# BurntSushi/rust-snappy

Hardware: AMD Instinct MI355X
Metric: GiB/s uncompressed (compress + decompress) on zflat/uflat corpus (higher is better)
Workload: dtype u8

## Files before the change

rust-snappy_amd/csrc/snapmi_api.hip:

```cpp
#include <hip/hip_runtime.h>

#include <cstdarg>
#include <cstdio>
#include <cstdlib>
#include <cstring>
#include <new>
#include <string>
#include <vector>

#include "snapmi.h"
#include "snapmi_test.h"
#include "snapmi_ctx.hpp"
#include "snapmi_launch.hpp"
#include "snapmi_device.hpp"
#include "snapmi_kernels.hpp"

using namespace snapmi;

namespace {

void set_err(snapmi_error *e, int kind, uint64_t a = 0, uint64_t b = 0,
             uint64_t c = 0)
{
    if (e) {
// ... 251 lines not shown
        ctx->lane_table_tries = (uint32_t)value;
    else if (strcmp(name, "lane_table_budget_pct") == 0 && value >= 1 &&
             value <= 90)
        ctx->lane_table_budget_pct = (uint32_t)value;
    else if (strcmp(name, "token_pool_pct") == 0 && value >= 1 &&
             value <= 100) {
        ctx->token_pool_pct = (uint32_t)value;
        ctx->token_pool_now = 0;
    } else if (strcmp(name, "token_pool_min_pages") == 0 && value >= 0 &&
               value <= 0x7FFFFFFF)
        ctx->token_pool_min_pages = (uint32_t)value;
    else if (strcmp(name, "span_schedule") == 0 && value >= 0 && value <= 2)
        ctx->span_schedule = (int)value;
    else if (strcmp(name, "lane_coresident") == 0 && value >= 0 && value <= 1)
        ctx->lane_coresident = (int)value;
    else if (strcmp(name, "lane_coresident_min_blocks") == 0 && value >= 1)
        ctx->lane_coresident_min_blocks = (uint64_t)value;
    else if (strcmp(name, "small_table_kernel") == 0 && value >= 0 &&
             value <= 1)
        ctx->small_table_kernel = (int)value;
    else if (strcmp(name, "small_table_min_blocks") == 0 && value >= 1)
        ctx->small_table_min_blocks = (uint64_t)value;
    else if (strcmp(name, "small_batch_kernel") == 0 && value >= 0 &&
             value <= 2)
        ctx->small_batch_kernel = (int)value;
    else if (strcmp(name, "lane_speculate") == 0 && value >= 0 && value <= 1)
        ctx->lane_speculate = (int)value;
    else if (strcmp(name, "lane_tail_probes") == 0 && value >= 0 &&
             value <= 4)
        ctx->lane_tail_probes = (uint32_t)value;
    else if (strcmp(name, "lane_tail_idle_pct") == 0 && value >= 0 &&
             value <= 100)
        ctx->lane_tail_idle_pct = (uint32_t)value;
    else if (strcmp(name, "span_kernel") == 0 && value >= kSpanMin &&
             value <= 1)
        ctx->span_kernel = (int)value;
    else if (strcmp(name, "match_kernel") == 0 && value >= 0 && value <= 2)
        ctx->match_kernel = (int)value;
    else if (strcmp(name, "match_spans_ratio_pct") == 0 && value >= 1 &&
             value <= 200)
        ctx->match_spans_ratio_pct = (uint32_t)value;
    else if (strcmp(name, "release_scratch") == 0 && value >= 0 && value <= 1)
        ctx->release_scratch = (int)value;
    else if (strcmp(name, "batch_long_streams") == 0 && value >= 0 &&
             value <= 1)
        ctx->batch_long_streams = (int)value;
    else if (strcmp(name, "both_wave_cus") == 0 && value >= 0 &&
             value <= 4096)
        ctx->both_wave_cus = (uint32_t)value;
    else if (strcmp(name, "tiny_stream_kernel") == 0 && value >= 0 &&
             value <= 1)
        ctx->tiny_stream_kernel = (int)value;
    else if (strcmp(name, "small_stream_kernel") == 0 && value >= 0 &&
             value <= 2)
        ctx->small_stream_kernel = (int)value;
    else if (strcmp(name, "frame_parallel_walk_min") == 0 && value >= 0)
        ctx->frame_parallel_walk_min = (uint64_t)value;
    else if (strcmp(name, "host_copy_kernel") == 0 && value >= 0 && value <= 3)
        ctx->host_copy_kernel = (int)value;
    else if (strcmp(name, "host_encode_slice") == 0 && value >= (1 << 16))
        ctx->host_encode_slice = (uint64_t)value;
    else if (strcmp(name, "host_decode_slice_chunks") == 0 && value >= 1)
        ctx->host_decode_slice_chunks = (uint64_t)value;
    else if (strcmp(name, "host_batch_slice") == 0 && value >= (1 << 16))
        ctx->host_batch_slice = (uint64_t)value;
    else if (strcmp(name, "range_scratch_bytes") == 0 && value >= (128 << 10))
// ... 42 lines not shown
             value <= 1)
        ctx->lane_table_probe = value != 0;
    else if (strcmp(name, "lane_tables_renew") == 0 && value == 1) {
        if (ctx->lane_tables.p) {
            HIP_TRY(ctx, hipStreamSynchronize(ctx->stream));
            snapmi::free_lane_tables(ctx);
        }
    } else if (strcmp(name, "lane_epoch_preset") == 0 && value >= -1 &&
             value <= 0xFFFF)
        ctx->lane_epoch_preset = value;
    else if (strcmp(name, "index_build_route") == 0 && value >= 0 &&
             value <= 2)
        ctx->index_build_route = (uint32_t)value;
    else if (strcmp(name, "index_build_group_streams") == 0 && value >= 1 &&
             value <= 4096)
        ctx->index_build_group_streams = (uint32_t)value;
    else if (strcmp(name, "stream_seg_log2") == 0 &&
             (value == 0 || value == 10 || value == 12))
        ctx->stream_seg_log2 = (uint32_t)value;
    else if (strcmp(name, "stream_scan_segs") == 0 &&
             (value == 0 || value == 8 || value == 16 || value == 32 ||
              value == 64))
        ctx->stream_scan_segs = (uint32_t)value;
    else if (strcmp(name, "lds_order_ok") == 0 && value >= 0 && value <= 1)
        ctx->lds_order_ok = ctx->lds_order_hw && value != 0;
    else if (strcmp(name, "host_batch_direct_min") == 0 && value >= 0)
        ctx->host_batch_direct_min = (uint64_t)value;
    else if (strcmp(name, "host_batch_pack_to_host") == 0 && value >= 0 &&
             value <= 1)
        ctx->host_batch_pack_to_host = (int)value;
    else if (strcmp(name, "host_batch_listed") == 0 && value >= 0 &&
             value <= 1)
        ctx->host_batch_listed = (int)value;
    else
        return fail_ctx(ctx, SNAPMI_E_ARGUMENT, "unknown test option %s",
                        name);
    return SNAPMI_OK;
}
#endif

void *snapmi_host_alloc(size_t bytes)
{
    void *p = nullptr;
    if (hipHostMalloc(&p, bytes ? bytes : 1, hipHostMallocDefault) != hipSuccess) {
        (void)hipGetLastError();
        return nullptr;
    }
    return p;
}

void snapmi_host_free(void *p)
{
    if (p)
        (void)hipHostFree(p);
}

const char *snapmi_table_probe_log(const snapmi_ctx *ctx)
{
    return ctx ? ctx->probe_log.c_str() : "";
}

size_t snapmi_error_string(const snapmi_error *e, char *buf, size_t cap)
{
    char tmp[256];
    const unsigned long long a = e ? e->a : 0, b = e ? e->b : 0,
                             c = e ? e->c : 0;
// ... 153 lines not shown
        return SNAPMI_TOO_BIG;
    }
    *result = (size_t)v;
    return SNAPMI_OK;
}

int snapmi_ctx_get_info(snapmi_ctx *ctx, const char *name, int64_t *value)
{
    if (!ctx || !name || !value)
        return SNAPMI_E_ARGUMENT;
    if (strcmp(name, "scratch_bytes") == 0) {
        uint64_t sum = ctx->lane_tables.cap;
        for (const DevBuf *b : ctx->dev_bufs)
            sum += b->cap;
        *value = (int64_t)sum;
    } else if (strcmp(name, "token_scratch_bytes") == 0) {
        *value = (int64_t)(ctx->tokens.cap + ctx->tok_pages.cap +
                           ctx->tok_stage.cap + ctx->ntok.cap);
    } else if (strcmp(name, "token_pool_pages") == 0) {
        *value = ctx->tok_pool_pages_last;
#ifdef SNAPMI_TESTING
    } else if (strcmp(name, "lane_multi_rounds") == 0) {
        uint32_t w = 0;
        if (ctx->tok_pages.p) {
            HIP_TRY(ctx, hipSetDevice(ctx->device));
            HIP_TRY(ctx, hipStreamSynchronize(ctx->stream));
            HIP_TRY(ctx, hipMemcpy(&w,
                                   (const uint32_t *)ctx->tok_pages.p +
                                       snapmi::kTokCtlMultiRounds,
                                   sizeof w, hipMemcpyDeviceToHost));
        }
        *value = w;
#endif
    } else if (strcmp(name, "token_pool_pct_now") == 0) {
        *value = ctx->token_pool_now;
    } else if (strcmp(name, "token_pages_asked") == 0 ||
               strcmp(name, "token_blocks_spilled") == 0) {
        HIP_TRY(ctx, hipSetDevice(ctx->device));
        HIP_TRY(ctx, hipStreamSynchronize(ctx->stream));
        const volatile uint32_t *t = ctx->h_tokstat;
        *value = !t ? 0 : name[6] == 'p' ? t[0] : t[1];
    } else if (strcmp(name, "index_streams_pieced") == 0 ||
               strcmp(name, "index_streams_fallback") == 0) {
        unsigned long long w[3] = {0, 0, 0};
        if (ctx->ix_stats_live && ctx->ix_gate.p) {
            HIP_TRY(ctx, hipSetDevice(ctx->device));
            HIP_TRY(ctx, hipStreamSynchronize(ctx->stream));
            HIP_TRY(ctx, hipMemcpy(w, ctx->ix_gate.p, sizeof w,
                                   hipMemcpyDeviceToHost));
        }
        *value = (int64_t)(name[14] == 'p' ? w[1] : w[2]);
    } else if (strcmp(name, "range_pieces") == 0) {
        *value = (int64_t)ctx->rg_pieces;
    } else if (strcmp(name, "range_ranges_ok") == 0 ||
               strcmp(name, "range_ranges_failed") == 0) {
        unsigned long long w[2] = {0, 0};
        if (ctx->rg_stats_live && ctx->rg_stat.p) {
            HIP_TRY(ctx, hipSetDevice(ctx->device));
            HIP_TRY(ctx, hipStreamSynchronize(ctx->stream));
            HIP_TRY(ctx, hipMemcpy(w, ctx->rg_stat.p, sizeof w,
                                   hipMemcpyDeviceToHost));
        }
        *value = (int64_t)(name[13] == 'o' ? w[0] : w[1]);
    } else if (strcmp(name, "write_blocks") == 0) {
        *value = (int64_t)ctx->wr_blocks;
    } else if (strcmp(name, "write_blocks_decoded") == 0) {
// ... 273 lines not shown
```

rust-snappy_amd/csrc/snapmi_compress.hip:

```cpp
#include <type_traits>

#include "snapmi_device.hpp"
#include "snapmi_kernels.hpp"
#include "snapmi_scan.hpp"
#include "snapmi_span.hpp"

namespace snapmi {

namespace {

__device__ __forceinline__ uint32_t hash32(uint32_t x, uint32_t shift)
{
    return (x * 0x1E35A7BDu) >> shift;
}

struct DeltaTable {
    uint32_t d[448];
};
constexpr DeltaTable make_delta()
{
    DeltaTable t{};
    uint32_t skip = 32, p = 0;
    for (int i = 0; i < 448; i++) {
        t.d[i] = p < 0x100000u ? p : 0x100000u;
// ... 1808 lines not shown
            m.out = (gptr)a.out_ptrs[st];
            a.out_lens[st] = tiny_compress(m, n);
        }
        __syncthreads();
    }
}
}
__global__ __launch_bounds__(64) void k_compress_small512(CompressArgs a)
{
    compress_small<512, 8>(a);
}
__global__ __launch_bounds__(64) void k_compress_small1k(CompressArgs a)
{
    compress_small<1024, 4>(a);
}
__global__ __launch_bounds__(64) void k_compress_small2k(CompressArgs a)
{
    compress_small<2048, 2>(a);
}

__device__ __forceinline__ uint32_t ld32p(gcptr p)
{
    uint32_t v;
    __builtin_memcpy(&v, p, 4);
    return v;
}
__device__ __forceinline__ uint64_t ld64p(gcptr p)
{
    uint64_t v;
    __builtin_memcpy(&v, p, 8);
    return v;
}
namespace {
constexpr uint32_t kLaneRingWords = 64 * 64;
constexpr uint32_t kLaneTokWords = 64 * 16;
template <bool kSpec, bool kTail>
__device__ __forceinline__ void match_blocks(
    const CompressArgs &a, const uint32_t lane, const uint32_t g,
    __attribute__((address_space(3))) uint32_t *const ring,
    __attribute__((address_space(3))) unsigned long long *const tokbuf)
{
    typedef __attribute__((address_space(3))) uint32_t l_tok;
    l_tok *const tbuf = (l_tok *)(tokbuf + lane * 16);
    typedef __attribute__((address_space(3))) uint32_t l_u32;
    typedef __attribute__((address_space(3))) u32x4 l_u32x4;
    typedef __attribute__((address_space(1))) u32x4 g_u32x4;
    l_u32 *const win = ring + lane * 64;

    typedef __attribute__((address_space(1))) unsigned long long g_u64;
    typedef unsigned long long u64x2 __attribute__((ext_vector_type(2)));
    typedef __attribute__((address_space(1))) u64x2 g_entry;
    const uint32_t slot =
        a.lane_chunks ? (g % a.lane_chunks) * a.lane_per_chunk + g / a.lane_chunks
                      : g;
    g_entry *const tab =
        (g_entry *)a.lane_tables + (uint64_t)slot * a.lane_stride;
    unsigned long long epoch = a.lane_epochs[g];
    unsigned long long first8 = 0;
    uint32_t first4b = 0;
    uint32_t nblocks = a.blk_first[a.n_streams];
    if (nblocks > a.host_blocks)
        nblocks = a.host_blocks;
    if (nblocks > a.blk_hi)
        nblocks = a.blk_hi;

    enum : uint32_t {
// ... 105 lines not shown
                out_of_work = true;
            } else {
                uint32_t lo = 0, hi_st = a.n_streams;
                if (b < a.n_streams && a.blk_first[b] == b && a.blk_first[b + 1] > b) {
                    lo = b;
                    hi_st = b + 1;
                }
                while (hi_st - lo > 1) {
                    const uint32_t mid = (lo + hi_st) >> 1;
                    if (a.blk_first[mid] <= b)
                        lo = mid;
                    else
                        hi_st = mid;
                }
                const uint32_t k = b - a.blk_first[lo];
                const uint64_t total = a.in_lens[lo];
                const uint64_t boff = (uint64_t)k * kMaxBlock;
                src = (gcptr)a.in_ptrs[lo] + boff;
                n = total - boff < kMaxBlock ? (uint32_t)(total - boff)
                                             : kMaxBlock;
                spilled = false;
                ntok = 0;
                nexc = 0;
                csize = 0;
                next_emit = 0;
                have = true;
                if (n <= a.cls_lo || n > a.cls_hi) {
                    have = false;
                } else if (n < kMinNonLiteral) {
                    g_tok *const at = tok_at(0);
                    if (!spilled)
                        *at = tok_pack(n, 0, 0);
                    a.ntok[b] = spilled ? kTokSpilled : 1u;
                    a.blk_size[b] = token_bytes(n, 0, 0);
                    have = false;
                } else {
                    first8 = ld64p(src);
                    first4b = ld32p(src + 8);
                    epoch = (epoch + 1) & 0xFFFFu;
                    if (epoch == 0) {
                        for (uint32_t i = 0; i < kMaxTable; i++)
                            tab[i] = (u64x2){0, 0};
                        epoch = 1;
                    }
                    shift = 32 - 8;
                    uint32_t tsize = 256;
                    while (tsize < kMaxTable && tsize < n) {
                        shift--;
                        tsize *= 2;
                    }
                    s_limit = n - kInputMargin;
                    s = 1;
                    s_next = 2;
                    skip = 33;
                    mode = kProbe;
                    mis = (uint32_t)(uintptr_t)src & 127u;
                    src_al = src - mis;
                    hi = 0;
                }
            }
        }
        if ((kTail || kProfTailBuild) && M_need) {
            const uint64_t M_out = __ballot(need && out_of_work);
            if (M_out) {
                if (kTail && lane == (uint32_t)__builtin_ctzll(M_out))
                    atomicAdd(&a.ticket[kTicketIdle],
                              (uint32_t)__builtin_popcountll(M_out));
// ... 269 lines not shown
            s_next = s + step;
            skip += step;
            mode = kProbe;
            if (s_next > s_limit)
                finished = true;
        }
        if (finished)
            flush = flush || (ntok & 31) != 0;
        if (flush) {
            g_u32x4 *to = (g_u32x4 *)tok_at((ntok - 1) & ~31u);
            const l_u32x4 *from = (const l_u32x4 *)tbuf;
            const u32x4 t0 = from[0], t1 = from[1], t2 = from[2], t3 = from[3],
                        t4 = from[4], t5 = from[5], t6 = from[6], t7 = from[7];
            if (!spilled) {
                to[0] = t0; to[1] = t1; to[2] = t2; to[3] = t3;
                to[4] = t4; to[5] = t5; to[6] = t6; to[7] = t7;
            }
        }
        if (finished) {
            if (next_emit < n) {
                const uint32_t tl = n - next_emit;
                g_tok *const at =
                    ntok % 32 ? (g_tok *)a.tok_pool +
                                    (uint64_t)tpage * kTokPage + ntok % kTokPage
                              : tok_at(ntok);
                if (!spilled)
                    *at = tok_pack(tl, 0, 0);
                ntok++;
                if (!tok_fits(tl, 0))
                    exc_put(tok_pack64(tl, 0, 0));
                csize += token_bytes(tl, 0, 0);
            }
            a.ntok[b] = spilled ? kTokSpilled : ntok;
            a.blk_size[b] = csize;
            have = false;
        }
    }
    a.lane_epochs[g] = epoch;
    PROF_TAIL(
    if (a.prof && lane == 0)
        atomicMax(&a.prof[kProfTail + 1], (unsigned long long)wall_clock64());
    )
#ifdef SNAPMI_TESTING
    if (kTail && lane == 0 && multi_rounds)
        atomicAdd(&a.tok_ctl[kTokCtlMultiRounds], multi_rounds);
#endif
}
}

#define SNAPMI_LANE_KERNEL(name, spec, tail)                                  \
    __global__ __launch_bounds__(64) void name(CompressArgs a)                \
    {                                                                         \
        __shared__ __attribute__((aligned(16))) uint32_t ring[kLaneRingWords]; \
        __shared__ __attribute__((aligned(16)))                               \
        unsigned long long tokbuf[kLaneTokWords];                             \
        match_blocks<spec, tail>(                                             \
            a, threadIdx.x, blockIdx.x * 64 + threadIdx.x,                    \
            (__attribute__((address_space(3))) uint32_t *)ring,               \
            (__attribute__((address_space(3))) unsigned long long *)tokbuf);  \
    }
SNAPMI_LANE_KERNEL(k_match_blocks, false, true)
SNAPMI_LANE_KERNEL(k_match_blocks_plain, false, false)
SNAPMI_LANE_KERNEL(k_match_blocks_spec, true, false)
#undef SNAPMI_LANE_KERNEL

namespace {
template <bool kTail>
__device__ __forceinline__ void match_both(
    const CompressArgs &a,
    __attribute__((address_space(3))) uint32_t *const ring,
    __attribute__((address_space(3))) unsigned long long *const tokbuf,
    const lptr16 tables)
{
    const uint32_t lane = threadIdx.x & 63;
    const uint32_t wave = uni(threadIdx.x >> 6);
    if (wave < kBothLaneWaves) {
        match_blocks<false, kTail>(
            a, lane, (blockIdx.x * kBothLaneWaves + wave) * 64 + lane,
            ring + wave * kLaneRingWords, tokbuf + wave * kLaneTokWords);
        return;
    }
    const lptr16 table = tables + (wave - kBothLaneWaves) * kMaxTable;
    const uint32_t tbase = (uint32_t)(uintptr_t)table;
    uint32_t nblocks = a.blk_first[a.n_streams];
    if (nblocks > a.host_blocks)
        nblocks = a.host_blocks;
    if (nblocks > a.blk_hi)
        nblocks = a.blk_hi;
    for (;;) {
        const uint32_t b =
            uni(next_back_ticket(a.ticket, lane, a.blk_lo, nblocks));
        if (b == 0xFFFFFFFFu)
            break;
        compress_one_block_span<false, true>(a, b, lane, table, tbase);
    }
    PROF_TAIL(
    if (a.prof && lane == 0)
        atomicMax(&a.prof[kProfTail + 1], (unsigned long long)wall_clock64());
    )
}
}
#define SNAPMI_BOTH_KERNEL(name, tail)                                        \
    __global__ __launch_bounds__(kBothWaves * 64) void name(CompressArgs a)   \
    {                                                                         \
        __shared__ __attribute__((aligned(16)))                               \
        uint32_t ring[kBothLaneWaves][kLaneRingWords];                        \
        __shared__ __attribute__((aligned(16)))                               \
        unsigned long long tokbuf[kBothLaneWaves][kLaneTokWords];             \
        __shared__ __attribute__((aligned(16)))                               \
        uint16_t tables[kBothWaves - kBothLaneWaves][kMaxTable];              \
        match_both<tail>(                                                     \
            a, (__attribute__((address_space(3))) uint32_t *)&ring[0][0],     \
            (__attribute__((address_space(3))) unsigned long long *)          \
                &tokbuf[0][0],                                                \
            (lptr16)&tables[0][0]);                                           \
    }
SNAPMI_BOTH_KERNEL(k_match_both, true)
SNAPMI_BOTH_KERNEL(k_match_both_plain, false)
#undef SNAPMI_BOTH_KERNEL

__global__ __launch_bounds__(64) void k_encode_tokens(CompressArgs a)
{
    const uint32_t lane = threadIdx.x;
    const uint32_t b = a.blk_lo + blockIdx.x;
    uint32_t nblocks = a.blk_first[a.n_streams];
    if (nblocks > a.host_blocks)
        nblocks = a.host_blocks;
    if (nblocks > a.blk_hi)
        nblocks = a.blk_hi;
    if (b >= nblocks)
        return;
    if (a.ntok[b] >= kTokSpilled)
        return;
    uint32_t lo = 0, hi = a.n_streams;
    if (b < a.n_streams && a.blk_first[b] == b && a.blk_first[b + 1] > b) {
        lo = b;
        hi = b + 1;
    }
    while (hi - lo > 1) {
        const uint32_t mid = (lo + hi) >> 1;
        if (a.blk_first[mid] <= b)
            lo = mid;
        else
            hi = mid;
    }
    const uint32_t st = lo;
    const uint32_t k = b - a.blk_first[st];
    const uint64_t total = a.in_lens[st];
    const uint64_t boff = (uint64_t)k * kMaxBlock;
    gcptr src = (gcptr)a.in_ptrs[st] + boff;
    const uint32_t n =
        total - boff < kMaxBlock ? (uint32_t)(total - boff) : kMaxBlock;
    gptr dst;
    if (k == 0) {
        dst = (gptr)a.out_ptrs[st];
        if (lane == 0) {
            uint64_t v = total;
            uint32_t i = 0;
            while (v >= 0x80) {
                dst[i++] = (uint8_t)v | 0x80;
                v >>= 7;
            }
            dst[i] = (uint8_t)v;
        }
        dst += varint_len(total);
    } else if (a.direct) {
        const uint32_t first = a.blk_first[st];
        const uint64_t nb = (total + kMaxBlock - 1) / kMaxBlock;
        if (first + nb > a.host_blocks)
            return;
        dst = (gptr)a.out_ptrs[st] + varint_len(total) +
              (a.blk_off[b] - a.blk_off[first]);
    } else {
        const uint32_t slot = a.slot_first[st] + k - 1;
        if (slot >= a.host_slots)
            return;
        dst = (gptr)a.scratch + (uint64_t)slot * kSlotBytes;
    }
    TokenSink out;
    out.init(src, n, dst, lane);
    typedef __attribute__((address_space(1))) uint32_t g_tok;
    typedef __attribute__((address_space(1))) unsigned long long g_u64;
    const uint32_t ptab =
        lane < kPageTabStride
            ? a.tok_pages[(uint64_t)(b - a.tok_base) * kPageTabStride + lane]
            : 0;
    const g_tok *const pool = (const g_tok *)a.tok_pool;
    const uint32_t count = a.ntok[b];
    uint32_t pos_base = 0, exc_base = 0;
    uint32_t tnext =
        lane < count ? pool[(uint64_t)rdlane(ptab, 0) * kTokPage + lane] : 0;
    for (uint32_t t0 = 0; t0 < count; t0 += kWave) {
        const uint32_t m = count - t0 < kWave ? count - t0 : kWave;
        uint32_t L = 0, C = 0, O = 0;
        const uint32_t t = tnext;
        if (t0 + kWave < count) {
            const uint32_t pg = rdlane(ptab, (t0 + kWave) / kTokPage);
            if (t0 + kWave + lane < count)
                tnext = pool[(uint64_t)pg * kTokPage +
                             (t0 + kWave) % kTokPage + lane];
        }
        const uint32_t field = (t >> 10) & 63u;
        if (lane < m) {
            L = t & 1023u;
            C = field == kTokLiteral ? 0u : field + 4u;
            O = t >> 16;
        }
        const bool ex = lane < m && field == kTokException;
        const uint64_t E = __builtin_amdgcn_ballot_w64(ex);
        if (E) {
            const uint32_t ei =
                exc_base + __builtin_amdgcn_mbcnt_hi(
                               (uint32_t)(E >> 32),
                               __builtin_amdgcn_mbcnt_lo((uint32_t)E, 0));
            const uint32_t eslot = ei / kExcPage < kExcPagesPerBlock
                                       ? ei / kExcPage
                                       : kExcPagesPerBlock - 1;
            const uint32_t epg = (uint32_t)__builtin_amdgcn_ds_bpermute(
                (int)((kTokPagesPerBlock + eslot) << 2), (int)ptab);
            if (ex) {
                const unsigned long long f =
                    ((const g_u64 *)(pool + (uint64_t)epg * kTokPage))
                        [ei % kExcPage];
                L = (uint32_t)f & 0x1FFFFu;
                C = (uint32_t)(f >> 17) & 0xFFFFu;
                O = (uint32_t)(f >> 33) & 0xFFFFu;
            }
            exc_base += (uint32_t)__builtin_popcountll(E);
        }
        const uint32_t span = L + C;
        const uint32_t incl = wave_inclusive_scan(span);
        const uint32_t P = pos_base + incl - span;
        pos_base += rdlane(incl, kWave - 1);
        out.a = (L & 0xFFFFu) | (O << 16);
        out.b = C | (P << 16);
        out.t = m;
        out.flush();
    }
    if (lane == 0 && !a.direct)
        a.blk_size[b] = out.d;
}

namespace {
__device__ __forceinline__ uint32_t plan_blocks(const CompressArgs &a,
                                                uint32_t i, bool report)
{
    const uint64_t len = a.in_lens[i];
    const uint64_t need = max_compress_len_u64(len);
    if (report)
        a.out_lens[i] = 0;
    if (need == 0) {
        if (report)
            set_error(a.errs, i, SNAPMI_TOO_BIG, len, kMaxInput, 0);
        return 0;
    }
    if (a.out_caps && a.out_caps[i] < need) {
        if (report)
            set_error(a.errs, i, SNAPMI_BUFFER_TOO_SMALL, a.out_caps[i], need,
                      0);
        return 0;
    }
    if (len == 0) {
        if (report) {
            ((gptr)a.out_ptrs[i])[0] = 0;
            a.out_lens[i] = 1;
            set_error(a.errs, i, SNAPMI_OK, 0, 0, 0);
        }
        return 0;
    }
    if (report)
        set_error(a.errs, i, SNAPMI_OK, 0, 0, 0);
    if (len < a.small_limit)
        return 0;
// ... 271 lines not shown
```

rust-snappy_amd/csrc/snapmi_ctx.hpp:

```cpp
#pragma once

#include <hip/hip_runtime.h>

#include <cstdarg>
#include <cstdio>
#include <string>
#include <vector>

#include "snapmi.h"

namespace snapmi {

struct DevBuf {
    void *p = nullptr;
    size_t cap = 0;
    bool listed = false;
};

struct PinBuf {
    void *p = nullptr;
    size_t cap = 0;
    bool listed = false;
};

// ... 26 lines not shown
    std::vector<hipMemGenericAllocationHandle_t> lane_chunks;
    size_t lane_chunk_bytes = 0, lane_va_bytes = 0;
    uint32_t lane_chunk_count = 0, lane_per_chunk = 0;
    uint32_t n_lanes = 0;
    uint64_t lane_stride = 0;
    bool lane_table_spread = true;
    bool lane_tables_top = false;
    int compress_mode = 1;
    int span_schedule = 1;
    snapmi::DevBuf sched;
    int lane_coresident = 1;
    uint64_t lane_coresident_min_blocks = 98304;
    const char *last_kernel = "";
    int small_table_kernel = 1;
    uint64_t small_table_min_blocks = 256;
    int small_batch_kernel = 1;
    int span_kernel = 1;
    uint32_t both_wave_cus = 0;
    int release_scratch = 0;
    int match_kernel = 2;
    uint32_t match_spans_ratio_pct = 90;
    volatile uint32_t *h_ratio = nullptr;
    uint32_t ratio_seq = 0;
    uint32_t token_pool_pct = 39, token_pool_now = 0;
    uint32_t token_pool_min_pages = 32768;
    volatile uint32_t *h_tokstat = nullptr;
    uint32_t tokstat_seq = 0, tokstat_seen = 0;
    uint32_t tok_pages_asked = 0, tok_blocks_spilled = 0;
    uint32_t tok_pool_pages_last = 0;
    int lane_speculate = 1;
    uint64_t lane_speculate_max_blocks = 24576;
    uint32_t lane_tail_probes = 2;
    uint32_t lane_tail_idle_pct = 40;
    int tiny_stream_kernel = 1;
    int small_stream_kernel = 1;
    uint64_t decode_many_min = 1u << 20;
    int lane_overlap_encode = 0;
    int lane_tables_uncached = 0;
    int decode_kernel = 3;
    hipStream_t stream2 = nullptr;
    hipEvent_t ev_fork = nullptr, ev_join = nullptr;
    hipEvent_t ev_crc[2] = {nullptr, nullptr};
    bool frame_crc_side_stream = true;
    snapmi::DevBuf st_in, st_out, st_desc, st_prof, ticket, order;
    snapmi::DevBuf sd_tables, sd_desc;
    int batch_long_streams = 1;
    snapmi::DevBuf bl_modes, bl_list, bl_descs, bl_order;
    snapmi::PinBuf pin_bl;
    snapmi::PinBuf pin_bl2;
    snapmi::DevBuf ix_modes, ix_desc, ix_gate;
    uint64_t ix_seq = 0;
    bool ix_stats_live = false;
    snapmi::DevBuf rg_desc, rg_meta, rg_part, rg_room, rg_stat;
    uint64_t range_scratch_bytes = 1ull << 30;
    uint64_t rg_pieces = 0;
    bool rg_stats_live = false;
    snapmi::DevBuf ib_meta, ib_stat;
    snapmi::PinBuf pin_ib, pin_ibg[2];
    hipEvent_t ev_ib = nullptr, ev_ibg[2] = {nullptr, nullptr};
    bool ev_ib_live = false, ev_ibg_live[2] = {false, false};
    uint64_t ib_groups = 0;
    bool ib_stats_live = false;
    snapmi::DevBuf wr_meta, wr_state, wr_z, wr_slot, wr_room, wr_desc, wr_stat;
    snapmi::PinBuf pin_wr;
    hipEvent_t ev_wr = nullptr;
    bool ev_wr_live = false;
// ... 87 lines not shown
```

rust-snappy_amd/csrc/snapmi_kernels.hpp:

```cpp
#pragma once

#include <hip/hip_runtime.h>
#include <stdint.h>

#include "snapmi.h"
#include "snapmi_tiny.hpp"
#include "snapmi_profile.hpp"
#include "snapmi_streamplan.hpp"
#include "snapmi_blockindex.hpp"

namespace snapmi {

struct CompressArgs {
    const void *const *in_ptrs;
    const uint64_t *in_lens;
    void *const *out_ptrs;
    const uint64_t *out_caps;
    uint64_t *out_lens;
    snapmi_error *errs;
    uint32_t *blk_first;
    uint32_t *slot_first;
    uint32_t *blk_size;
    uint64_t *blk_off;
    uint8_t *scratch;
    uint32_t n_streams;
    uint32_t host_blocks;
    uint32_t host_slots;
    uint32_t *ticket;
    uint32_t *sched;
    uint32_t *tok_pool;
    uint32_t *tok_pages;
    uint32_t *tok_ctl;
    uint32_t tok_pool_pages;
    uint32_t *tok_stage;
    uint32_t tok_stage_waves, tok_stage_wave0;
    uint32_t *ntok;
    uint32_t blk_lo, blk_hi;
    uint32_t tok_base;
    uint32_t direct;
    unsigned long long *lane_tables;
    unsigned long long lane_stride;
    uint32_t lane_chunks, lane_per_chunk;
    uint32_t *lane_epochs;
    uint32_t n_lanes;
    uint32_t lane_depth, lane_tail_depth, lane_tail_idle;
    unsigned long long *prof;
    uint2 *plan_part;
    unsigned long long *scan_part;
    uint32_t small_limit;
    uint32_t cls_lo, cls_hi;
};

constexpr uint32_t kCompressWaves = 5;
constexpr uint32_t kSmallTableWaves = 10;
#define SNAPMI_BOTH_WAVES 6
#define SNAPMI_BOTH_LANE_WAVES 4
constexpr uint32_t kBothWaves = SNAPMI_BOTH_WAVES,
                   kBothLaneWaves = SNAPMI_BOTH_LANE_WAVES;
constexpr uint32_t kMaxTokens = 16416;
constexpr uint32_t kTokPage = 512, kExcPage = 256;
constexpr uint32_t kTokPagesPerBlock = (kMaxTokens + kTokPage - 1) / kTokPage;
constexpr uint32_t kExcPagesPerBlock = 4;
constexpr uint32_t kPageTabStride = 40;
static_assert(kTokPagesPerBlock + kExcPagesPerBlock <= kPageTabStride, "");
constexpr uint32_t kPagesPerSmallBlock = (8192 / 4 + 64 + kTokPage - 1) / kTokPage + 1;
constexpr uint32_t kTokCtlList = 16;
constexpr uint32_t kProfTail = 16, kProfTailLanes = 32;
constexpr uint32_t kTicketIdle = 2;
constexpr uint32_t kTokCtlMultiRounds = 4;
constexpr uint32_t kTokStageWords = kMaxTokens + 2 * (kMaxTokens / 16) + 28;
constexpr uint32_t kTokSpilled = 0xFFFFFFFEu;
constexpr uint32_t kTokLiteral = 61, kTokException = 62;
#if defined(__HIPCC__)
__device__ __forceinline__ bool tok_fits(uint32_t lit, uint32_t copy)
{
    return lit <= 1023u && copy <= 64u;
}
__device__ __forceinline__ uint32_t tok_pack(uint32_t lit, uint32_t copy,
                                             uint32_t offset)
{
    const uint32_t field = copy ? copy - 4u : kTokLiteral;
    return tok_fits(lit, copy) ? (offset << 16) | (field << 10) | lit
                               : kTokException << 10;
}
__device__ __forceinline__ unsigned long long tok_pack64(uint32_t lit,
                                                         uint32_t copy,
                                                         uint32_t offset)
{
    return (unsigned long long)lit | ((unsigned long long)copy << 17) |
           ((unsigned long long)offset << 33);
}
#endif

struct DecompressArgs {
    const void *const *in_ptrs;
    const uint64_t *in_lens;
    void *const *out_ptrs;
    const uint64_t *out_caps;
    uint64_t *out_lens;
    snapmi_error *errs;
    const uint8_t *modes;
    const unsigned long long *gate;
// ... 316 lines not shown
```

rust-snappy_amd/csrc/snapmi_launch.hip:

```cpp
#include <hip/hip_runtime.h>

#include <cstdio>
#include <cstring>
#include <vector>

#include "snapmi.h"
#include "snapmi_test.h"
#include "snapmi_ctx.hpp"
#include "snapmi_launch.hpp"
#include "snapmi_pool.hpp"
#include "snapmi_route.hpp"
#include "snapmi_device.hpp"
#include "snapmi_kernels.hpp"

using namespace snapmi;

namespace snapmi {
static_assert(kRouteCompressWaves == kCompressWaves &&
                  kRouteSmallTableWaves == kSmallTableWaves &&
                  kRouteBothWaves == kBothWaves &&
                  kRouteBothLaneWaves == kBothLaneWaves &&
                  kRouteTinyCompress == kTinyCompress &&
                  kRouteSmallCompress == kSmallCompress,
              "snapmi_route.hpp and snapmi_kernels.hpp disagree");
// ... 259 lines not shown
    a.in_lens = d_in_lens;
    a.out_ptrs = d_out_ptrs;
    a.out_caps = d_out_caps;
    a.out_lens = d_out_lens;
    a.errs = d_errs;
    a.blk_first = (uint32_t *)ctx->blk_first.p;
    a.slot_first = (uint32_t *)ctx->slot_first.p;
    a.blk_size = (uint32_t *)ctx->blk_size.p;
    a.blk_off = (uint64_t *)ctx->blk_off.p;
    a.plan_part = (uint2 *)ctx->plan_part.p;
    a.scan_part = (unsigned long long *)ctx->plan_part.p;
    a.n_streams = (uint32_t)n;
    a.host_blocks = (uint32_t)blocks;
    a.host_slots = (uint32_t)slots;
    a.ticket = (uint32_t *)ctx->ticket.p;
    a.tok_pool = nullptr;
    a.tok_pages = nullptr;
    a.tok_ctl = nullptr;
    a.tok_pool_pages = 0;
    a.tok_stage = nullptr;
    a.tok_stage_waves = 0;
    a.tok_stage_wave0 = 0;
    a.sched = nullptr;
    a.ntok = nullptr;
    a.lane_tables = nullptr;
    a.lane_epochs = nullptr;
    a.lane_stride = kMaxTable;
    a.lane_chunks = 0;
    a.lane_per_chunk = 0;
    a.n_lanes = 0;
    a.lane_depth = 1;
    a.lane_tail_depth = 0;
    a.lane_tail_idle = 0;
    a.tok_base = 0;
    a.small_limit = (uint32_t)small_stream_limit(o);
    a.cls_lo = 0;
    a.cls_hi = kMaxBlock;
    a.direct = route.direct ? 1 : 0;
    if (!route.direct &&
        (rc = reserve(ctx, ctx->slots, (slots + 1) * (size_t)kSlotBytes)))
        return rc;
    a.scratch = (uint8_t *)ctx->slots.p;
    a.blk_lo = 0;
    a.blk_hi = (uint32_t)blocks;
    if (ctx->h_tokstat) {
        const volatile uint32_t *t = ctx->h_tokstat;
        const uint32_t seq = t[3];
        if (seq != ctx->tokstat_seen) {
            ctx->tokstat_seen = seq;
            const uint32_t asked = t[0], spilled = t[1], of = t[2];
            if (t[3] == seq && of) {
                ctx->tok_pages_asked = asked;
                ctx->tok_blocks_spilled = spilled;
                ctx->token_pool_now =
                    snapmi::pool_grow(ctx->token_pool_now, spilled, of);
            }
        }
    }
    if (ctx->token_pool_now < ctx->token_pool_pct)
        ctx->token_pool_now = ctx->token_pool_pct;
    const uint64_t pool_pages =
        snapmi::pool_pages(block_bytes, blocks, route.seg_blocks, route.lanes,
                           ctx->token_pool_now, ctx->token_pool_min_pages);
    const size_t pool_bytes = (size_t)(pool_pages + 1) * kTokPage * 4;
    const size_t stage_bytes =
        (size_t)ctx->num_cus * route.stage_waves * kTokStageWords * 4;
// ... 105 lines not shown
        if (route.window_beside) {
            HIP_TRY(ctx, hipEventRecord(ctx->ev_fork, s));
            HIP_TRY(ctx, hipStreamWaitEvent(ctx->stream2, ctx->ev_fork, 0));
            ws = ctx->stream2;
        }
        if (route.sched) {
            const size_t head = (size_t)(16 + n) * 4;
            const size_t lists = (size_t)2 * (slots + 1) * 4;
            if ((rc = reserve(ctx, ctx->sched, head + lists)))
                return rc;
            HIP_TRY(ctx, hipMemsetAsync(ctx->sched.p, 0, head, ws));
            HIP_TRY(ctx, hipMemsetAsync((uint8_t *)ctx->sched.p + head, 0xFF,
                                        lists, ws));
            a.sched = (uint32_t *)ctx->sched.p;
        }
        launch_window(route, a, ws);
        a.sched = nullptr;
    }
    if (route.tokens) {
        HIP_TRY(ctx, hipEventRecord(ctx->ev[4], s));
        for (uint64_t lo = 0; lo < blocks; lo += route.seg_blocks) {
            const uint64_t hi = lo + route.seg_blocks < blocks
                                    ? lo + route.seg_blocks
                                    : blocks;
            const Segment g = segment(o, route, lo, hi);
            a.tok_base = (uint32_t)lo;
            a.blk_lo = (uint32_t)lo;
            a.blk_hi = (uint32_t)g.mid;
            HIP_TRY(ctx, hipMemsetAsync(ctx->tok_pages.p, 0,
                                        kTokCtlList * 4, s));
            if (route.window == WindowKernel::none)
                HIP_TRY(ctx, hipMemsetAsync(ctx->ticket.p, 0, 64, s));
            a.cls_lo = route.small_grid ? 8192 : 0;
            launch_match(o, route, g, a, s);
            if (route.small_grid) {
                HIP_TRY(ctx, hipMemsetAsync(ctx->ticket.p, 0, 64, s));
                a.cls_lo = 0;
                a.cls_hi = 8192;
                hipLaunchKernelGGL(k_match_spans_8k, dim3(route.small_grid),
                                   dim3(kSmallTableWaves * 64), 0, s, a);
            }
            a.cls_lo = 0;
            a.cls_hi = kMaxBlock;
            if (g.mid < hi) {
                HIP_TRY(ctx, hipEventRecord(ctx->ev_fork, s));
                HIP_TRY(ctx,
                        hipStreamWaitEvent(ctx->stream2, ctx->ev_fork, 0));
                hipLaunchKernelGGL(k_encode_tokens,
                                   dim3((uint32_t)(g.mid - lo)), dim3(64), 0,
                                   ctx->stream2, a);
                HIP_TRY(ctx, hipEventRecord(ctx->ev_join, ctx->stream2));
                a.blk_lo = (uint32_t)g.mid;
                a.blk_hi = (uint32_t)hi;
                HIP_TRY(ctx, hipMemsetAsync(ctx->ticket.p, 0, 64, s));
                launch_match(o, route, g, a, s);
            }
            if (hi == blocks)
                HIP_TRY(ctx, hipEventRecord(ctx->ev[5], s));
            if (route.window_beside) {
                HIP_TRY(ctx, hipEventRecord(ctx->ev_join, ctx->stream2));
                HIP_TRY(ctx, hipStreamWaitEvent(s, ctx->ev_join, 0));
            }
            if (route.direct)
                launch_scan_sizes(a, s);
            hipLaunchKernelGGL(k_encode_tokens,
                               dim3((uint32_t)(hi - a.blk_lo)), dim3(64), 0, s,
                               a);
// ... 173 lines not shown
```

Baseline: 123.8.

## Encode tokens inside the combined match kernel's tail once predecessor sizes are known

After: 124.6, median of 4. Within noise of the previous version (+0.7%).

```diff
diff --git a/rust-snappy_amd/csrc/snapmi_api.hip b/rust-snappy_amd/csrc/snapmi_api.hip
--- a/rust-snappy_amd/csrc/snapmi_api.hip
+++ b/rust-snappy_amd/csrc/snapmi_api.hip
@@ -307,6 +307,8 @@
     else if (strcmp(name, "lane_tail_idle_pct") == 0 && value >= 0 &&
              value <= 100)
         ctx->lane_tail_idle_pct = (uint32_t)value;
+    else if (strcmp(name, "tail_encode") == 0 && value >= 0 && value <= 1)
+        ctx->tail_encode = (int)value;
     else if (strcmp(name, "span_kernel") == 0 && value >= kSpanMin &&
              value <= 1)
         ctx->span_kernel = (int)value;
@@ -415,6 +417,9 @@
     else if (strcmp(name, "host_batch_listed") == 0 && value >= 0 &&
              value <= 1)
         ctx->host_batch_listed = (int)value;
+    else if (strcmp(name, "tail_list_cap") == 0 && value >= 0 &&
+             value <= 0x7FFFFFFF)
+        ctx->tail_list_cap = (uint32_t)value;
     else
         return fail_ctx(ctx, SNAPMI_E_ARGUMENT, "unknown test option %s",
                         name);
@@ -634,6 +639,20 @@
         }
         *value = w;
 #endif
+    } else if (strcmp(name, "tail_encoded_blocks") == 0 ||
+               strcmp(name, "tail_encode_skipped") == 0) {
+        uint32_t w = 0;
+        if (ctx->tok_pages.p) {
+            HIP_TRY(ctx, hipSetDevice(ctx->device));
+            HIP_TRY(ctx, hipStreamSynchronize(ctx->stream));
+            HIP_TRY(ctx, hipMemcpy(&w,
+                                   (const uint32_t *)ctx->tok_pages.p +
+                                       (name[11] == 'd'
+                                            ? snapmi::kTokCtlTailEncoded
+                                            : snapmi::kTokCtlTailSkipped),
+                                   sizeof w, hipMemcpyDeviceToHost));
+        }
+        *value = w;
     } else if (strcmp(name, "token_pool_pct_now") == 0) {
         *value = ctx->token_pool_now;
     } else if (strcmp(name, "token_pages_asked") == 0 ||
diff --git a/rust-snappy_amd/csrc/snapmi_compress.hip b/rust-snappy_amd/csrc/snapmi_compress.hip
--- a/rust-snappy_amd/csrc/snapmi_compress.hip
+++ b/rust-snappy_amd/csrc/snapmi_compress.hip
@@ -1864,6 +1864,28 @@
     return v;
 }
 namespace {
+template <bool kAgent>
+__device__ __forceinline__ void publish_size(const CompressArgs &a,
+                                             uint32_t b, uint32_t size)
+{
+    if (kAgent)
+        __hip_atomic_store(&a.blk_size[b], size, __ATOMIC_RELAXED,
+                           __HIP_MEMORY_SCOPE_AGENT);
+    else
+        a.blk_size[b] = size;
+}
+__device__ __forceinline__ void tail_append(const CompressArgs &a, uint32_t b,
+                                            bool second_look)
+{
+    uint32_t *const ctl = a.tail_ctl + blockIdx.x * kTailCtlWords;
+    __builtin_amdgcn_fence(__ATOMIC_RELEASE, "workgroup");
+    const uint32_t at = __hip_atomic_fetch_add(
+        &ctl[kTailAppended], 1u, __ATOMIC_RELAXED, __HIP_MEMORY_SCOPE_AGENT);
+    if (at < a.tail_cap)
+        __hip_atomic_store(&a.tail_list[(uint64_t)blockIdx.x * a.tail_cap + at],
+                           tail_entry(b, second_look), __ATOMIC_RELAXED,
+                           __HIP_MEMORY_SCOPE_AGENT);
+}
 constexpr uint32_t kLaneRingWords = 64 * 64;
 constexpr uint32_t kLaneTokWords = 64 * 16;
 template <bool kSpec, bool kTail>
@@ -2035,7 +2057,7 @@
                     if (!spilled)
                         *at = tok_pack(n, 0, 0);
                     a.ntok[b] = spilled ? kTokSpilled : 1u;
-                    a.blk_size[b] = token_bytes(n, 0, 0);
+                    publish_size<kTail>(a, b, token_bytes(n, 0, 0));
                     have = false;
                 } else {
                     first8 = ld64p(src);
@@ -2371,10 +2393,15 @@
                 csize += token_bytes(tl, 0, 0);
             }
             a.ntok[b] = spilled ? kTokSpilled : ntok;
-            a.blk_size[b] = csize;
+            publish_size<kTail>(a, b, csize);
+            if (kTail && a.tail_ctl && !spilled)
+                tail_append(a, b, false);
             have = false;
         }
     }
+    if (kTail && a.tail_ctl && lane == 0)
+        atomicAdd(&a.tail_ctl[blockIdx.x * kTailCtlWords + kTailLanesDone],
+                  1u);
     a.lane_epochs[g] = epoch;
     PROF_TAIL(
     if (a.prof && lane == 0)
@@ -2404,73 +2431,9 @@
 #undef SNAPMI_LANE_KERNEL
 
 namespace {
-template <bool kTail>
-__device__ __forceinline__ void match_both(
-    const CompressArgs &a,
-    __attribute__((address_space(3))) uint32_t *const ring,
-    __attribute__((address_space(3))) unsigned long long *const tokbuf,
-    const lptr16 tables)
-{
-    const uint32_t lane = threadIdx.x & 63;
-    const uint32_t wave = uni(threadIdx.x >> 6);
-    if (wave < kBothLaneWaves) {
-        match_blocks<false, kTail>(
-            a, lane, (blockIdx.x * kBothLaneWaves + wave) * 64 + lane,
-            ring + wave * kLaneRingWords, tokbuf + wave * kLaneTokWords);
-        return;
-    }
-    const lptr16 table = tables + (wave - kBothLaneWaves) * kMaxTable;
-    const uint32_t tbase = (uint32_t)(uintptr_t)table;
-    uint32_t nblocks = a.blk_first[a.n_streams];
-    if (nblocks > a.host_blocks)
-        nblocks = a.host_blocks;
-    if (nblocks > a.blk_hi)
-        nblocks = a.blk_hi;
-    for (;;) {
-        const uint32_t b =
-            uni(next_back_ticket(a.ticket, lane, a.blk_lo, nblocks));
-        if (b == 0xFFFFFFFFu)
-            break;
-        compress_one_block_span<false, true>(a, b, lane, table, tbase);
-    }
-    PROF_TAIL(
-    if (a.prof && lane == 0)
-        atomicMax(&a.prof[kProfTail + 1], (unsigned long long)wall_clock64());
-    )
-}
-}
-#define SNAPMI_BOTH_KERNEL(name, tail)                                        \
-    __global__ __launch_bounds__(kBothWaves * 64) void name(CompressArgs a)   \
-    {                                                                         \
-        __shared__ __attribute__((aligned(16)))                               \
-        uint32_t ring[kBothLaneWaves][kLaneRingWords];                        \
-        __shared__ __attribute__((aligned(16)))                               \
-        unsigned long long tokbuf[kBothLaneWaves][kLaneTokWords];             \
-        __shared__ __attribute__((aligned(16)))                               \
-        uint16_t tables[kBothWaves - kBothLaneWaves][kMaxTable];              \
-        match_both<tail>(                                                     \
-            a, (__attribute__((address_space(3))) uint32_t *)&ring[0][0],     \
-            (__attribute__((address_space(3))) unsigned long long *)          \
-                &tokbuf[0][0],                                                \
-            (lptr16)&tables[0][0]);                                           \
-    }
-SNAPMI_BOTH_KERNEL(k_match_both, true)
-SNAPMI_BOTH_KERNEL(k_match_both_plain, false)
-#undef SNAPMI_BOTH_KERNEL
-
-__global__ __launch_bounds__(64) void k_encode_tokens(CompressArgs a)
-{
-    const uint32_t lane = threadIdx.x;
-    const uint32_t b = a.blk_lo + blockIdx.x;
-    uint32_t nblocks = a.blk_first[a.n_streams];
-    if (nblocks > a.host_blocks)
-        nblocks = a.host_blocks;
-    if (nblocks > a.blk_hi)
-        nblocks = a.blk_hi;
-    if (b >= nblocks)
-        return;
-    if (a.ntok[b] >= kTokSpilled)
-        return;
+__device__ __forceinline__ uint32_t block_stream(const CompressArgs &a,
+                                                 uint32_t b)
+{
     uint32_t lo = 0, hi = a.n_streams;
     if (b < a.n_streams && a.blk_first[b] == b && a.blk_first[b + 1] > b) {
         lo = b;
@@ -2483,14 +2446,17 @@
         else
             hi = mid;
     }
-    const uint32_t st = lo;
-    const uint32_t k = b - a.blk_first[st];
-    const uint64_t total = a.in_lens[st];
+    return lo;
+}
+__device__ __forceinline__ uint32_t encode_block_tokens(
+    const CompressArgs &a, const uint32_t b, const uint32_t lane,
+    const uint32_t st, const uint32_t k, const uint64_t total,
+    const uint32_t count, gptr dst)
+{
     const uint64_t boff = (uint64_t)k * kMaxBlock;
     gcptr src = (gcptr)a.in_ptrs[st] + boff;
     const uint32_t n =
         total - boff < kMaxBlock ? (uint32_t)(total - boff) : kMaxBlock;
-    gptr dst;
     if (k == 0) {
         dst = (gptr)a.out_ptrs[st];
         if (lane == 0) {
@@ -2503,18 +2469,6 @@
             dst[i] = (uint8_t)v;
         }
         dst += varint_len(total);
-    } else if (a.direct) {
-        const uint32_t first = a.blk_first[st];
-        const uint64_t nb = (total + kMaxBlock - 1) / kMaxBlock;
-        if (first + nb > a.host_blocks)
-            return;
-        dst = (gptr)a.out_ptrs[st] + varint_len(total) +
-              (a.blk_off[b] - a.blk_off[first]);
-    } else {
-        const uint32_t slot = a.slot_first[st] + k - 1;
-        if (slot >= a.host_slots)
-            return;
-        dst = (gptr)a.scratch + (uint64_t)slot * kSlotBytes;
     }
     TokenSink out;
     out.init(src, n, dst, lane);
@@ -2525,7 +2479,6 @@
             ? a.tok_pages[(uint64_t)(b - a.tok_base) * kPageTabStride + lane]
             : 0;
     const g_tok *const pool = (const g_tok *)a.tok_pool;
-    const uint32_t count = a.ntok[b];
     uint32_t pos_base = 0, exc_base = 0;
     uint32_t tnext =
         lane < count ? pool[(uint64_t)rdlane(ptab, 0) * kTokPage + lane] : 0;
@@ -2576,8 +2529,193 @@
         out.t = m;
         out.flush();
     }
+    return out.d;
+}
+
+__device__ __forceinline__ void tail_encode(const CompressArgs &a,
+                                            const uint32_t lane)
+{
+    uint32_t *const ctl = a.tail_ctl + blockIdx.x * kTailCtlWords;
+    const uint32_t *const list =
+        a.tail_list + (uint64_t)blockIdx.x * a.tail_cap;
+    auto peek = [&](const uint32_t *p) -> uint32_t {
+        return uni(__hip_atomic_load(p, __ATOMIC_RELAXED,
+                                     __HIP_MEMORY_SCOPE_AGENT));
+    };
+    uint32_t encoded = 0, skipped = 0;
+    for (;;) {
+        if (peek(&ctl[kTailLanesDone]) >= kBothLaneWaves)
+            break;
+        uint32_t at = 0;
+        if (lane == 0)
+            at = __hip_atomic_fetch_add(&ctl[kTailTaken], 1u, __ATOMIC_RELAXED,
+                                        __HIP_MEMORY_SCOPE_AGENT);
+        at = uni(at);
+        if (at >= a.tail_cap)
+            break;
+        uint32_t e;
+        while ((e = peek(&list[at])) == 0) {
+            if (peek(&ctl[kTailLanesDone]) >= kBothLaneWaves)
+                break;
+            __builtin_amdgcn_s_sleep(127);
+            __builtin_amdgcn_s_sleep(127);
+            __builtin_amdgcn_s_sleep(127);
+        }
+        if (e == 0)
+            break;
+        __builtin_amdgcn_fence(__ATOMIC_ACQUIRE, "workgroup");
+        const uint32_t b = tail_entry_block(e);
+        const uint32_t count = a.ntok[b];
+        if (count >= kTokSpilled)
+            continue;
+        const uint32_t st = block_stream(a, b);
+        const uint32_t first = a.blk_first[st];
+        const uint32_t k = b - first;
+        const uint64_t total = a.in_lens[st];
+        const uint64_t nb = (total + kMaxBlock - 1) / kMaxBlock;
+        uint64_t off = 0;
+        const TailLook look =
+            (uint64_t)first + nb > a.host_blocks
+                ? TailLook::too_far
+                : tail_look(
+                      k,
+                      [&](uint32_t i) -> uint32_t {
+                          return __hip_atomic_load(&a.blk_size[first + i],
+                                                   __ATOMIC_RELAXED,
+                                                   __HIP_MEMORY_SCOPE_AGENT);
+                      },
+                      &off);
+        if (uni((uint32_t)look) != (uint32_t)TailLook::ready) {
+            if (look == TailLook::not_ready && !tail_entry_second_look(e)) {
+                if (lane == 0)
+                    tail_append(a, b, true);
+            } else {
+                skipped++;
+            }
+            continue;
+        }
+        off = uni64(off);
+        encode_block_tokens(a, b, lane, st, k, total, count,
+                            (gptr)a.out_ptrs[st] + varint_len(total) + off);
+        if (lane == 0)
+            a.ntok[b] = 0xFFFFFFFFu;
+        encoded++;
+    }
+    if (lane == 0) {
+        if (encoded)
+            atomicAdd(&a.tok_ctl[kTokCtlTailEncoded], encoded);
+        if (skipped)
+            atomicAdd(&a.tok_ctl[kTokCtlTailSkipped], skipped);
+    }
+}
+}
+
+namespace {
+template <bool kTail>
+__device__ __forceinline__ void match_both(
+    const CompressArgs &a,
+    __attribute__((address_space(3))) uint32_t *const ring,
+    __attribute__((address_space(3))) unsigned long long *const tokbuf,
+    const lptr16 tables)
+{
+    const uint32_t lane = threadIdx.x & 63;
+    const uint32_t wave = uni(threadIdx.x >> 6);
+    if (wave < kBothLaneWaves) {
+        match_blocks<false, kTail>(
+            a, lane, (blockIdx.x * kBothLaneWaves + wave) * 64 + lane,
+            ring + wave * kLaneRingWords, tokbuf + wave * kLaneTokWords);
+        return;
+    }
+    const lptr16 table = tables + (wave - kBothLaneWaves) * kMaxTable;
+    const uint32_t tbase = (uint32_t)(uintptr_t)table;
+    uint32_t nblocks = a.blk_first[a.n_streams];
+    if (nblocks > a.host_blocks)
+        nblocks = a.host_blocks;
+    if (nblocks > a.blk_hi)
+        nblocks = a.blk_hi;
+    for (;;) {
+        const uint32_t b =
+            uni(next_back_ticket(a.ticket, lane, a.blk_lo, nblocks));
+        if (b == 0xFFFFFFFFu)
+            break;
+        compress_one_block_span<false, true>(a, b, lane, table, tbase);
+        if (kTail && a.tail_ctl) {
+            __builtin_amdgcn_fence(__ATOMIC_RELEASE, "workgroup");
+            uint32_t size = kTailSizeUnknown, count = kTokSpilled;
+            if (lane == 0) {
+                size = a.blk_size[b];
+                count = a.ntok[b];
+            }
+            if (size != kTailSizeUnknown) {
+                publish_size<true>(a, b, size);
+                if (count < kTokSpilled)
+                    tail_append(a, b, false);
+            }
+        }
+    }
+    if (kTail && a.tail_ctl)
+        tail_encode(a, lane);
+    PROF_TAIL(
+    if (a.prof && lane == 0)
+        atomicMax(&a.prof[kProfTail + 1], (unsigned long long)wall_clock64());
+    )
+}
+}
+#define SNAPMI_BOTH_KERNEL(name, tail)                                        \
+    __global__ __launch_bounds__(kBothWaves * 64) void name(CompressArgs a)   \
+    {                                                                         \
+        __shared__ __attribute__((aligned(16)))                               \
+        uint32_t ring[kBothLaneWaves][kLaneRingWords];                        \
+        __shared__ __attribute__((aligned(16)))                               \
+        unsigned long long tokbuf[kBothLaneWaves][kLaneTokWords];             \
+        __shared__ __attribute__((aligned(16)))                               \
+        uint16_t tables[kBothWaves - kBothLaneWaves][kMaxTable];              \
+        match_both<tail>(                                                     \
+            a, (__attribute__((address_space(3))) uint32_t *)&ring[0][0],     \
+            (__attribute__((address_space(3))) unsigned long long *)          \
+                &tokbuf[0][0],                                                \
+            (lptr16)&tables[0][0]);                                           \
+    }
+SNAPMI_BOTH_KERNEL(k_match_both, true)
+SNAPMI_BOTH_KERNEL(k_match_both_plain, false)
+#undef SNAPMI_BOTH_KERNEL
+
+__global__ __launch_bounds__(64) void k_encode_tokens(CompressArgs a)
+{
+    const uint32_t lane = threadIdx.x;
+    const uint32_t b = a.blk_lo + blockIdx.x;
+    uint32_t nblocks = a.blk_first[a.n_streams];
+    if (nblocks > a.host_blocks)
+        nblocks = a.host_blocks;
+    if (nblocks > a.blk_hi)
+        nblocks = a.blk_hi;
+    if (b >= nblocks)
+        return;
+    const uint32_t count = a.ntok[b];
+    if (count >= kTokSpilled)
+        return;
+    const uint32_t st = block_stream(a, b);
+    const uint32_t k = b - a.blk_first[st];
+    const uint64_t total = a.in_lens[st];
+    gptr dst = nullptr;
+    if (k == 0) {
+    } else if (a.direct) {
+        const uint32_t first = a.blk_first[st];
+        const uint64_t nb = (total + kMaxBlock - 1) / kMaxBlock;
+        if (first + nb > a.host_blocks)
+            return;
+        dst = (gptr)a.out_ptrs[st] + varint_len(total) +
+              (a.blk_off[b] - a.blk_off[first]);
+    } else {
+        const uint32_t slot = a.slot_first[st] + k - 1;
+        if (slot >= a.host_slots)
+            return;
+        dst = (gptr)a.scratch + (uint64_t)slot * kSlotBytes;
+    }
+    const uint32_t size =
+        encode_block_tokens(a, b, lane, st, k, total, count, dst);
     if (lane == 0 && !a.direct)
-        a.blk_size[b] = out.d;
+        a.blk_size[b] = size;
 }
 
 namespace {
diff --git a/rust-snappy_amd/csrc/snapmi_ctx.hpp b/rust-snappy_amd/csrc/snapmi_ctx.hpp
--- a/rust-snappy_amd/csrc/snapmi_ctx.hpp
+++ b/rust-snappy_amd/csrc/snapmi_ctx.hpp
@@ -82,6 +82,9 @@
     uint64_t lane_speculate_max_blocks = 24576;
     uint32_t lane_tail_probes = 2;
     uint32_t lane_tail_idle_pct = 40;
+    int tail_encode = 1;
+    snapmi::DevBuf tail;
+    uint32_t tail_list_cap = 0;
     int tiny_stream_kernel = 1;
     int small_stream_kernel = 1;
     uint64_t decode_many_min = 1u << 20;
diff --git a/rust-snappy_amd/csrc/snapmi_kernels.hpp b/rust-snappy_amd/csrc/snapmi_kernels.hpp
--- a/rust-snappy_amd/csrc/snapmi_kernels.hpp
+++ b/rust-snappy_amd/csrc/snapmi_kernels.hpp
@@ -8,6 +8,7 @@
 #include "snapmi_profile.hpp"
 #include "snapmi_streamplan.hpp"
 #include "snapmi_blockindex.hpp"
+#include "snapmi_tailenc.hpp"
 
 namespace snapmi {
 
@@ -44,6 +45,8 @@
     uint32_t *lane_epochs;
     uint32_t n_lanes;
     uint32_t lane_depth, lane_tail_depth, lane_tail_idle;
+    uint32_t *tail_ctl, *tail_list;
+    uint32_t tail_cap;
     unsigned long long *prof;
     uint2 *plan_part;
     unsigned long long *scan_part;
@@ -68,6 +71,10 @@
 constexpr uint32_t kProfTail = 16, kProfTailLanes = 32;
 constexpr uint32_t kTicketIdle = 2;
 constexpr uint32_t kTokCtlMultiRounds = 4;
+constexpr uint32_t kTokCtlTailEncoded = 5, kTokCtlTailSkipped = 6;
+static_assert(kTokCtlTailSkipped < kTokCtlList, "");
+constexpr uint32_t kTailCtlWords = 16;
+constexpr uint32_t kTailAppended = 0, kTailTaken = 1, kTailLanesDone = 2;
 constexpr uint32_t kTokStageWords = kMaxTokens + 2 * (kMaxTokens / 16) + 28;
 constexpr uint32_t kTokSpilled = 0xFFFFFFFEu;
 constexpr uint32_t kTokLiteral = 61, kTokException = 62;
diff --git a/rust-snappy_amd/csrc/snapmi_launch.hip b/rust-snappy_amd/csrc/snapmi_launch.hip
--- a/rust-snappy_amd/csrc/snapmi_launch.hip
+++ b/rust-snappy_amd/csrc/snapmi_launch.hip
@@ -315,6 +315,9 @@
     a.lane_depth = 1;
     a.lane_tail_depth = 0;
     a.lane_tail_idle = 0;
+    a.tail_ctl = nullptr;
+    a.tail_list = nullptr;
+    a.tail_cap = 0;
     a.tok_base = 0;
     a.small_limit = (uint32_t)small_stream_limit(o);
     a.cls_lo = 0;
@@ -486,7 +489,29 @@
             if (route.window == WindowKernel::none)
                 HIP_TRY(ctx, hipMemsetAsync(ctx->ticket.p, 0, 64, s));
             a.cls_lo = route.small_grid ? 8192 : 0;
+            const bool tail_enc = ctx->tail_encode && route.direct &&
+                                  route.match == MatchKernel::both &&
+                                  a.lane_tail_depth > 1 && g.mid == hi;
+            if (tail_enc) {
+                const uint32_t wgs = match_grid(o, route, hi - lo);
+                const uint32_t cap =
+                    ctx->tail_list_cap
+                        ? ctx->tail_list_cap
+                        : snapmi::tail_list_entries(hi - lo, wgs);
+                const size_t bytes =
+                    (size_t)wgs * (kTailCtlWords + (size_t)cap) * 4;
+                if ((rc = reserve(ctx, ctx->tail, bytes)))
+                    return rc;
+                HIP_TRY(ctx, hipMemsetAsync(ctx->tail.p, 0, bytes, s));
+                HIP_TRY(ctx, hipMemsetAsync(a.blk_size + lo, 0xFF,
+                                            (size_t)(hi - lo) * 4, s));
+                a.tail_ctl = (uint32_t *)ctx->tail.p;
+                a.tail_list = a.tail_ctl + (size_t)wgs * kTailCtlWords;
+                a.tail_cap = cap;
+            }
             launch_match(o, route, g, a, s);
+            a.tail_ctl = nullptr;
+            a.tail_list = nullptr;
             if (route.small_grid) {
                 HIP_TRY(ctx, hipMemsetAsync(ctx->ticket.p, 0, 64, s));
                 a.cls_lo = 0;
diff --git a/rust-snappy_amd/csrc/snapmi_tailenc.hpp b/rust-snappy_amd/csrc/snapmi_tailenc.hpp
--- /dev/null
+++ b/rust-snappy_amd/csrc/snapmi_tailenc.hpp
@@ -0,0 +1,59 @@
+#pragma once
+#include <cstdint>
+
+#if defined(__HIPCC__)
+#define SNAPMI_TE_HD __host__ __device__ __forceinline__
+#else
+#define SNAPMI_TE_HD inline
+#endif
+
+namespace snapmi {
+
+constexpr uint32_t kTailSizeUnknown = 0xFFFFFFFFu;
+constexpr uint32_t kTailMaxPred = 64;
+
+constexpr uint32_t kTailSecondLook = 0x80000000u;
+SNAPMI_TE_HD uint32_t tail_entry(uint32_t block, bool second_look)
+{
+    return (block + 1u) | (second_look ? kTailSecondLook : 0u);
+}
+SNAPMI_TE_HD uint32_t tail_entry_block(uint32_t entry)
+{
+    return (entry & ~kTailSecondLook) - 1u;
+}
+SNAPMI_TE_HD bool tail_entry_second_look(uint32_t entry)
+{
+    return (entry & kTailSecondLook) != 0;
+}
+
+SNAPMI_TE_HD uint32_t tail_list_entries(uint64_t blocks, uint32_t cus)
+{
+    const uint64_t share = cus ? (blocks + cus - 1) / cus : blocks;
+    return (uint32_t)(2 * share + 64);
+}
+
+enum class TailLook : uint8_t {
+    ready,
+    not_ready,
+    too_far,
+};
+
+template <class SizeOf>
+SNAPMI_TE_HD TailLook tail_look(uint32_t k, SizeOf size_of, uint64_t *offset)
+{
+    if (k > kTailMaxPred)
+        return TailLook::too_far;
+    uint64_t sum = 0;
+    bool known = true;
+    for (uint32_t i = 0; i < k; i++) {
+        const uint32_t s = size_of(i);
+        known = known && s != kTailSizeUnknown;
+        sum += s;
+    }
+    if (!known)
+        return TailLook::not_ready;
+    *offset = sum;
+    return TailLook::ready;
+}
+
+}
```
